# gruai/koifish

Measured on AMD Instinct MI355X. Metric: tokens/sec/GPU Qwen3 4-bit prefill+decode; achieved HBM GB/s vs peak, higher is better.
Workload: dtype u4 weights x bf16, fp32 accumulate; 1 GPU; Qwen3-0.6B 4-bit PackedQ greedy decode, 1xMI355X per replica, seq=2048: prompt 128, timed positions 1996..2047; order=canonical: bit-exact vs the CPU oracle, lm_head=bf16, replicas=1

## Files before the change

koifish_amd/csrc/kf_abi.hip:

```cpp
#include <stdarg.h>
#include <stdio.h>
#include <string.h>


#include <mutex>
#include <math.h>
#include <stdlib.h>

#include <vector>

#include "kf_a8.h"
#include "kf_attn_plan.h"
#include "kf_attn_docs_plan.h"
#include "kf_gemm_plan.h"
#include "kf_gemv_plan.h"
#include "kf_gemv_rows_plan.h"
#include "kf_score_plan.h"
#include "kf_gama_plan.h"
#include "kf_lora_plan.h"
#include "kf_gradnorm_plan.h"
#include "kf_rowq.h"
#include "kf_engine_host.h"

struct kf_ctx {
// ... 1727 lines not shown
}
size_t kf_engine_head_screen_bytes(int vocab, int dim) { return kf::head_screen_bytes(vocab, dim); }
int kf_engine_set_head_screen(kf_ctx* c, kf_engine* e, void* buf, size_t bytes) {
    ENG_ENTER(c, e && e->h, "engine");
    ENG_NOT_CAPTURING(c);
    return ok_or(kf::engine_set_head_screen(e->h, buf, bytes, c->stream),
                 "kf_engine_set_head_screen: needs a head set by kf_engine_set_head and a 256-byte aligned buffer of kf_engine_head_screen_bytes(vocab, dim) bytes");
}
int kf_engine_screen_stats(kf_ctx* c, kf_engine* e, kf_engine_screen_statistics* out) {
    ENG_ENTER(c, e && e->h && out, "argument");
    long long w[3];
    ENG_HIP(kf::engine_screen_stats(e->h, c->stream, w));
    out->screened_steps = w[0], out->rows_reranked = w[1], out->wg_fallbacks = w[2];
    return KF_OK;
}
int kf_engine_reset(kf_ctx* c, kf_engine* e) {
    ENG_ENTER(c, e && e->h, "engine");
    ENG_NOT_CAPTURING(c);
    ENG_HIP(kf::eng_then_sync(KF_OK, c->stream));
    ENG_HIP(kf::engine_reset(e->h, c->stream));
    return KF_OK;
}
int kf_engine_set_embedding(kf_ctx* c, kf_engine* e, const kf_weight* embed_or_null, const int32_t* d_forced) {
    ENG_ENTER(c, e && e->h, "engine");
    ENG_NOT_CAPTURING(c);
    return ok_or(kf::engine_set_embedding(e->h, embed_or_null, d_forced),
                 "kf_engine_set_embedding: the fused row read takes a bf16 table of the engine's width (other storages keep kf_embed_state)");
}
int kf_engine_served(kf_ctx* c, const kf_engine_desc* d, char* why, size_t why_bytes) {
    CHKCTX(c);
    const char* w = "";
    const int rc = kf::engine_build(d, nullptr, 0, c->stream, nullptr, &w, kf::ENG_DRY);
    return eng_served(rc, __func__, w, why, why_bytes);
}
int kf_engine_tune(kf_ctx* c, kf_engine* e, kf_bf16* x_out, const int32_t* d_state, int pos_bound, int passes, float* us_before, float* us_after) {
    ENG_ENTER(c, e && e->h, "engine");
    ENG_NOT_CAPTURING(c);
    kf::engine_set_canonical(e->h, c->canonical);
    const int rc = kf::engine_tune(e->h, c->stream, x_out, d_state, pos_bound, passes, us_before, us_after);
    return rc < 0 ? fail(rc, "kf_engine_tune failed with %d (no embedding table set, or a poll timed out)", rc) : rc;
}
int kf_engine_stats(kf_ctx* c, kf_engine* e, int pos_bound, kf_engine_statistics* out) {
    ENG_ENTER(c, e && e->h && out, "argument");
    int w[14];
    ENG_HIP(kf::engine_stats(e->h, c->stream, pos_bound, w));
    for (int i = 0; i < 6; i++) out->sweeps[i] = w[i], out->delay[i] = w[7 + i];
    out->polls = w[6], out->tuned = w[13];
    return KF_OK;
}
int kf_engine_check(kf_ctx* c, kf_engine* e) {
    ENG_ENTER(c, e && e->h, "engine");
    int err = 0;
    ENG_HIP(kf::engine_error_word(e->h, c->stream, &err));
    if (err) return fail(KF_INTERNAL_ERR, "kf_engine: a hand-off poll timed out (error word 0x%x): the launch was not fully resident", err);
    return KF_OK;
}
size_t kf_xengine_workspace_bytes(const kf_engine_desc* d) { return d ? kf::xengine_ws_bytes(d) : 0; }
int kf_xengine_create(kf_ctx* c, const kf_engine_desc* d, int n_seq, int64_t kv_seq_stride, void* ws, size_t ws_bytes, kf_xengine** out) {
    ENG_ENTER(c, d && ws && out, "argument");
    ENG_NOT_CAPTURING(c);
    if (n_seq < 1 || n_seq > KF_XENGINE_MAX_SEQ) return fail(KF_INVALID_ARGS, "kf_xengine_create: n_seq %d outside 1 .. %d (up to four sequences per XCD)", n_seq, KF_XENGINE_MAX_SEQ);
    kf::XEngineHost* h = nullptr;
    const char* why = "";
    const int rc = kf::xengine_build(d, n_seq, (long long)kv_seq_stride, ws, ws_bytes, c->stream, &h, &why);
    return ENG_WRAP(kf_xengine, rc, why, h, out);
}
size_t kf_xengine_workspace_bytes_tp(const kf_engine_desc* d) { return d ? kf::xengine_ws_bytes_tp(d) : 0; }
int kf_xengine_create_tp(kf_ctx* c, const kf_engine_desc* const* ds, int world, void* ws, size_t ws_bytes, kf_xengine** out) {
    ENG_ENTER(c, ds && ws && out, "argument");
    ENG_NOT_CAPTURING(c);
    kf::XEngineHost* h = nullptr;
    const char* why = "";
    const int rc = kf::xengine_build_tp(ds, world, ws, ws_bytes, c->stream, &h, &why);
    return ENG_WRAP(kf_xengine, rc, why, h, out);
}
int kf_xengine_set_head_tp(kf_ctx* c, kf_xengine* e, const kf_weight* const* shards, const int32_t* row0, const kf_bf16* final_norm_w, kf_bf16* logits, int32_t* d_tokens_out, int tokens_stride) {
    ENG_ENTER(c, e && e->h, "engine");
    return ok_or(kf::xengine_set_head_tp(e->h, shards, row0, final_norm_w, logits, d_tokens_out, tokens_stride),
                 "kf_xengine_set_head_tp: eight bf16 [rows, dim] vocabulary shards in rank order (row0 = the rows before), a norm weight and a logits buffer");
}
int kf_xengine_served(kf_ctx* c, const kf_engine_desc* d, char* why, size_t why_bytes) {
    CHKCTX(c);
    if (!d) return fail(KF_INVALID_ARGS, "kf_xengine_served: null descriptor");
    const char* w = "";
    const int rc = kf::xengine_build(d, 1, 0, nullptr, 0, c->stream, nullptr, &w, kf::ENG_DRY);
    return eng_served(rc, __func__, w, why, why_bytes);
}
int kf_xengine_set_embedding(kf_ctx* c, kf_xengine* e, const kf_weight* embed, const int32_t* d_forced, int forced_stride) {
    ENG_ENTER(c, e && e->h && embed, "argument");
    if (d_forced && forced_stride < 1) return fail(KF_INVALID_ARGS, "kf_xengine_set_embedding: forced_stride %d", forced_stride);
    return ok_or(kf::xengine_set_embedding(e->h, embed, d_forced, forced_stride), "kf_xengine_set_embedding: the row read inside the launch takes a bf16 table of the engine's width");
}
int kf_xengine_set_head(kf_ctx* c, kf_xengine* e, const kf_weight* head_or_null, const kf_bf16* final_norm_w, kf_bf16* logits, int32_t* d_tokens_out, int tokens_stride) {
    ENG_ENTER(c, e && e->h, "engine");
    return ok_or(kf::xengine_set_head(e->h, head_or_null, final_norm_w, logits, d_tokens_out, tokens_stride),
                 "kf_xengine_set_head: the in-launch head takes a bf16 [vocab, dim] matrix of the engine's width, a norm weight and a logits buffer");
}
int kf_xengine_steps(kf_ctx* c, kf_xengine* e, kf_bf16* x_out, int32_t* d_state, int n_steps, int pick) {
    ENG_ENTER(c, e && e->h, "engine");
    if (!c->canonical) return fail(KF_UNSUPPORTED_DATATYPE, "kf_xengine_steps: the XCD-confined engines run the canonical summation order only (kf_set_canonical(ctx, 1))");
    if (n_steps < 1 || (n_steps > 1 && !pick)) return fail(KF_INVALID_ARGS, "kf_xengine_steps: n_steps %d (several steps per launch need the pick inside)", n_steps);
    if (c->capturing) return fail(KF_INVALID_ARGS, "kf_xengine_steps: not while capturing (the launch's generation is a kernel argument the host counts: a replayed launch would repeat it)");
    const int rc = kf::xengine_steps(e->h, c->stream, d_state, x_out, pick ? 2 : 1, n_steps);
    if (rc == KF_UNSUPPORTED_DATATYPE) return fail(rc, "kf_xengine_steps: the form for this many sequences does not fit the LDS at this depth");
    return rc == KF_OK ? KF_OK : fail(rc, "kf_xengine_steps failed with %d (no embedding / head set?)", rc);
}
// ... 212 lines not shown
```

koifish_amd/csrc/kf_attn_common.h:

```cpp
#pragma once
#include "kf_kernels.h"

namespace kf {

__device__ __forceinline__ float group_sum16(float v, int lg) {
    if (lg >= 1) v += dpp_f<0xB1>(v);
    if (lg >= 2) v += dpp_f<0x4E>(v);
    if (lg >= 3) v += dpp_f<0x141>(v);
    if (lg >= 4) v += dpp_f<0x140>(v);
    return v;
}
struct HeadRaw {
    uint16_t x0, x1, w0, w1;
};
__device__ __forceinline__ HeadRaw load_head(const uint16_t* __restrict__ src, const uint16_t* __restrict__ wn, int hd) {
    const int half = hd >> 1;
    int j = threadIdx.x & 63;
    j = j < half ? j : half - 1;
    const uint16_t* w = wn ? wn : src;
    return HeadRaw{src[j], src[j + half], w[j], w[j + half]};
}
__device__ __forceinline__ void prep_head_cs(const HeadRaw r, bool norm, bool rope, float c, float sn, int hd, float eps, uint16_t* dst, float* rstd_out = nullptr, int lane_in = -1) {
    const int lane = lane_in >= 0 ? lane_in : (int)(threadIdx.x & 63), half = hd >> 1;
    const int j = lane;
    const bool act = j < half;
    float x0 = act ? bf2f(r.x0) : 0.f, x1 = act ? bf2f(r.x1) : 0.f;
    if (norm) {
        const float w0 = bf2f(r.w0), w1 = bf2f(r.w1);
        const double ss = wave_sum_f64_fast(fma((double)x0, (double)x0, (double)x1 * (double)x1));
        const float s0 = 1.0f / sqrtf((float)ss / (float)hd + eps);
        const float s = round_bf16(s0);
        if (rstd_out && lane == 0) *rstd_out = s0;
        x0 = round_bf16(x0 * s * w0);
        x1 = round_bf16(x1 * s * w1);
    }
    if (rope) {
        const float a = x0 * c, b = x1 * sn, cc = x0 * sn, d = x1 * c;
        x0 = round_bf16(a - b);
        x1 = round_bf16(cc + d);
    }
    if (act) dst[j] = f2bf(x0), dst[j + half] = f2bf(x1);
}
__device__ __forceinline__ void prep_head(const HeadRaw r, bool norm, const float* __restrict__ tab_pos, int hd, float eps, uint16_t* dst, float* rstd_out = nullptr) {
    const int j = threadIdx.x & 63;
    float c = 1.f, sn = 0.f;
    if (tab_pos && j < (hd >> 1)) c = tab_pos[2 * j], sn = tab_pos[2 * j + 1];
    prep_head_cs(r, norm, tab_pos != nullptr, c, sn, hd, eps, dst, rstd_out);
}

__device__ __forceinline__ float fast_exp(float x) { return __builtin_amdgcn_exp2f(x * 1.44269502162933349609375f); }

constexpr int ATTN_U = 4;

struct AttnAt { int pos, t1; bool empty; };
template <int GQ, int NW, int HD, int EL>
struct AttnSlice {
    static constexpr int hd_log2 = HD == 128 ? 7 : 6;
    static constexpr int LPK = HD / EL, KPW = 64 / LPK, lpk_log2 = hd_log2 - (EL == 16 ? 4 : 3), tstride = NW * KPW, NQ = (GQ + NW - 1) / NW;
    const int gq_split, split, kvh, gpart, chunk, t0;
    __device__ __forceinline__ AttnSlice(int gq_split_, int chunk_)
        : gq_split(gq_split_), split(blockIdx.x), kvh((int)blockIdx.y / gq_split), gpart((int)blockIdx.y - kvh * gq_split), chunk(chunk_), t0(split * chunk) {}
    __device__ __forceinline__ int h0() const { return (kvh * gq_split + gpart) * GQ; }
    __device__ __forceinline__ int tstart(int wave, int grp) const { return t0 + wave * KPW + grp; }
    __device__ __forceinline__ int end(int last) const {
        int t = t0 + chunk;
        if (t > last + 1) t = last + 1;
        return t;
    }
    __device__ __forceinline__ AttnAt at(const int* d_pos, int pos_bound) const {
        const int pos = d_pos ? *d_pos : pos_bound, len = pos + 1;
        return AttnAt{pos, end(pos), t0 >= len};
    }
    __device__ __forceinline__ bool holds(int pos, int t1) const { return (pos >= t0) && (pos < t1); }
};

constexpr float KF_LOG2E = 1.44269502162933349609375f;
__device__ __forceinline__ float canon_score(const float (&q)[8], u32x4 kw, int lpk_log2, float rden) {
    const uint32_t k4[4] = {kw.x, kw.y, kw.z, kw.w};
    float d = 0.f;
#pragma unroll
    for (int i = 0; i < 4; i++) {
        d = fmaf(q[2 * i], bf_lo(k4[i]), d);
        d = fmaf(q[2 * i + 1], bf_hi(k4[i]), d);
    }
    d = group_sum16(d, lpk_log2);
    return round_bf16(d * rden);
}
__device__ __forceinline__ int canon_shift(float d) { return (int)fmaxf(d, -1022.0f); }
__device__ __forceinline__ double ldexp_d(double v, int e) { return __builtin_ldexp(v, e); }
__device__ __forceinline__ double swap32_add_d(double a, double b) {
    const unsigned long long ua = __builtin_bit_cast(unsigned long long, a), ub = __builtin_bit_cast(unsigned long long, b);
    const auto lo = __builtin_amdgcn_permlane32_swap((unsigned)ua, (unsigned)ub, false, false);
    const auto hi = __builtin_amdgcn_permlane32_swap((unsigned)(ua >> 32), (unsigned)(ub >> 32), false, false);
    return __builtin_bit_cast(double, ((unsigned long long)hi[0] << 32) | lo[0]) + __builtin_bit_cast(double, ((unsigned long long)hi[1] << 32) | lo[1]);
}
__device__ __forceinline__ double swap16_add_d(double a, double b) {
    const unsigned long long ua = __builtin_bit_cast(unsigned long long, a), ub = __builtin_bit_cast(unsigned long long, b);
    const auto lo = __builtin_amdgcn_permlane16_swap((unsigned)ua, (unsigned)ub, false, false);
    const auto hi = __builtin_amdgcn_permlane16_swap((unsigned)(ua >> 32), (unsigned)(ub >> 32), false, false);
    return __builtin_bit_cast(double, ((unsigned long long)hi[0] << 32) | lo[0]) + __builtin_bit_cast(double, ((unsigned long long)hi[1] << 32) | lo[1]);
}
template <int GQ>
struct CanonAcc {
    double o[GQ][8], l[GQ];
    float m[GQ];
    __device__ __forceinline__ void init() {
#pragma unroll
        for (int hq = 0; hq < GQ; hq++) {
            m[hq] = -__builtin_inff(), l[hq] = 0.0;
#pragma unroll
            for (int i = 0; i < 8; i++) o[hq][i] = 0.0;
        }
    }
};
template <int K>
__device__ __forceinline__ uint32_t row_bcast_u(uint32_t v) {
    return (uint32_t)__builtin_amdgcn_update_dpp(0, (int)v, 0x150 + K, 0xF, 0xF, true);
}
template <int K>
__device__ __forceinline__ float row_bcast_f(float v) { return __uint_as_float(row_bcast_u<K>(__float_as_uint(v))); }
template <int K>
__device__ __forceinline__ double row_bcast_d(double v) {
    const unsigned long long u = __builtin_bit_cast(unsigned long long, v);
    return __builtin_bit_cast(double, ((unsigned long long)row_bcast_u<K>((uint32_t)(u >> 32)) << 32) | row_bcast_u<K>((uint32_t)u));
}
__device__ __forceinline__ float canon_dot(const float (&q)[8], u32x4 kw, int lpk_log2) {
    const uint32_t k4[4] = {kw.x, kw.y, kw.z, kw.w};
    float d = 0.f;
#pragma unroll
// ... 78 lines not shown
        const double p = vmine ? ldexp_d((double)f, canon_shift(n - m_mine)) : 0.0;
        double vd[U][8];
#pragma unroll
        for (int u = 0; u < U; u++) {
            const uint32_t vw[4] = {vv[u].x, vv[u].y, vv[u].z, vv[u].w};
#pragma unroll
            for (int i = 0; i < 4; i++) vd[u][2 * i] = (double)bf_lo(vw[i]), vd[u][2 * i + 1] = (double)bf_hi(vw[i]);
        }
        canon_apply_items<GQ, U>(A, p, vd);
        return;
    }
    float f[U][GQ], n[U][GQ], bn[GQ];
#pragma unroll
    for (int hq = 0; hq < GQ; hq++) bn[hq] = -__builtin_inff();
#pragma unroll
    for (int u = 0; u < U; u++) {
#pragma unroll
        for (int hq = 0; hq < GQ; hq++) {
            const float s = canon_score(qf[hq], kk[u], lpk_log2, rden);
            kf_exp2_parts(s * KF_LOG2E, f[u][hq], n[u][hq]);
            n[u][hq] = valid[u] ? n[u][hq] : -__builtin_inff();
            bn[hq] = fmaxf(bn[hq], n[u][hq]);
        }
    }
#pragma unroll
    for (int hq = 0; hq < GQ; hq++) {
        bn[hq] = xmax32(xmax16(bn[hq]));
        if (LPK < 16) bn[hq] = fmaxf(bn[hq], dpp_f<0x128>(bn[hq]));
        if (bn[hq] > A.m[hq]) {
            if (A.m[hq] > -__builtin_inff()) {
                const int e = canon_shift(A.m[hq] - bn[hq]);
                A.l[hq] = ldexp_d(A.l[hq], e);
#pragma unroll
                for (int i = 0; i < 8; i++) A.o[hq][i] = ldexp_d(A.o[hq][i], e);
            }
            A.m[hq] = bn[hq];
        }
    }
#pragma unroll
    for (int u = 0; u < U; u++) {
        const uint32_t vw[4] = {vv[u].x, vv[u].y, vv[u].z, vv[u].w};
        double vd[8];
#pragma unroll
        for (int i = 0; i < 4; i++) vd[2 * i] = (double)bf_lo(vw[i]), vd[2 * i + 1] = (double)bf_hi(vw[i]);
#pragma unroll
        for (int hq = 0; hq < GQ; hq++) {
            const double p = valid[u] ? ldexp_d((double)f[u][hq], canon_shift(n[u][hq] - A.m[hq])) : 0.0;
            A.l[hq] += p;
#pragma unroll
            for (int i = 0; i < 8; i++) A.o[hq][i] = fma(p, vd[i], A.o[hq][i]);
        }
    }
}
template <int GQ, int LPK>
__device__ __forceinline__ void canon_wave_to_lds(const CanonAcc<GQ>& A, double* comb_wave , int hd, int lane, int d0) {
    const int row = lane >> 4;
#pragma unroll
    for (int hq = 0; hq < GQ; hq++) {
        double s1[4], r2[2];
#pragma unroll
        for (int i = 0; i < 4; i++) s1[i] = swap32_add_d(A.o[hq][i], A.o[hq][i + 4]);
#pragma unroll
        for (int i = 0; i < 2; i++) {
            r2[i] = swap16_add_d(s1[i], s1[i + 2]);
            if (LPK < 16) r2[i] += dpp_d<0x128>(r2[i]);
        }
        double lt = xsum16_d(xsum32_d(A.l[hq]));
        if (LPK < 16) lt += dpp_d<0x128>(lt);
        double* c = comb_wave + (size_t)hq * (hd + 2);
        if (LPK == 16 || (lane & 8) == 0) c[d0 + 2 * row] = r2[0], c[d0 + 2 * row + 1] = r2[1];
        if (lane == 0) c[hd] = lt, c[hd + 1] = (double)A.m[hq];
    }
}

template <int GQ, int NW, int HD>
__device__ __forceinline__ void canon_slice_publish(const double* comb, double* part, uint16_t* odst, int h0, int nsp, int split) {
    constexpr int hd = HD, hd_log2 = HD == 128 ? 7 : 6, PS = hd + 2;
    for (int i = threadIdx.x; i < GQ * hd; i += blockDim.x) {
        const int hq = i >> hd_log2, d = i & (hd - 1);
        float ms = -__builtin_inff();
#pragma unroll
        for (int sl = 0; sl < NW; sl++) ms = fmaxf(ms, (float)comb[((size_t)sl * GQ + hq) * PS + hd + 1]);
        double o = 0.0, L = 0.0;
#pragma unroll
        for (int sl = 0; sl < NW; sl++) {
            const double* c = comb + ((size_t)sl * GQ + hq) * PS;
            const int e = canon_shift((float)c[hd + 1] - ms);
            o += ldexp_d(c[d], e);
            L += ldexp_d(c[hd], e);
        }
        if (nsp == 1) {
            odst[(size_t)(h0 + hq) * hd + d] = f2bf((float)(o / L));
        } else {
            double* dst = part + ((size_t)(h0 + hq) * nsp + split) * PS;
            __hip_atomic_store(dst + d, o, __ATOMIC_RELAXED, __HIP_MEMORY_SCOPE_AGENT);
            if (d == 0) __hip_atomic_store(dst + hd, L, __ATOMIC_RELAXED, __HIP_MEMORY_SCOPE_AGENT), __hip_atomic_store(dst + hd + 1, (double)ms, __ATOMIC_RELAXED, __HIP_MEMORY_SCOPE_AGENT);
        }
    }
}
template <int GQ, int HD>
__device__ __forceinline__ void canon_slice_publish_empty(double* part, int h0, int nsp, int split) {
    constexpr int hd = HD, hd_log2 = HD == 128 ? 7 : 6, PS = hd + 2;
    for (int i = threadIdx.x; i < GQ * hd; i += blockDim.x) {
        const int hq = i >> hd_log2, d = i & (hd - 1);
        double* dst = part + ((size_t)(h0 + hq) * nsp + split) * PS;
        __hip_atomic_store(dst + d, 0.0, __ATOMIC_RELAXED, __HIP_MEMORY_SCOPE_AGENT);
        if (d == 0) __hip_atomic_store(dst + hd, 0.0, __ATOMIC_RELAXED, __HIP_MEMORY_SCOPE_AGENT), __hip_atomic_store(dst + hd + 1, -(double)__builtin_inff(), __ATOMIC_RELAXED, __HIP_MEMORY_SCOPE_AGENT);
    }
}
template <int GQ, int NW, int HD>
__device__ __forceinline__ void canon_arrive_and_merge(const double* part, int* counter, int* flag, uint16_t* odst, int h0, int nsp) {
    constexpr int hd = HD, hd_log2 = HD == 128 ? 7 : 6, PS = hd + 2;
    const int tid = threadIdx.x, lane = tid & 63;
    asm volatile("s_waitcnt vmcnt(0)" ::: "memory");
    __syncthreads();
    if (tid == 0) {
        const int old = __hip_atomic_fetch_add(counter, 1, __ATOMIC_RELAXED, __HIP_MEMORY_SCOPE_AGENT);
        flag[0] = (old == nsp - 1);
    }
    __syncthreads();
    if (!flag[0]) return;
    constexpr int NT = NW * 64;
    constexpr int NV = (GQ * 128 + NT - 1) / NT;
#pragma unroll
// ... 134 lines not shown
```

koifish_amd/csrc/kf_engine.hip:

```cpp
#include <stdlib.h>
#include <string.h>

#include <vector>

#include <type_traits>

#include "kf_attn_plan.h"
#include "kf_engine_common.h"
#include "kf_engine_host.h"

namespace kf {


struct EngXOff {
    int xA, qkv, ao, xB, act, part, hbest, tokg, end;
};
constexpr EngXOff eng_xoff(int dim, int qd, int kvd, int ffn, int hd) {
    EngXOff o{};
    o.xA = 0, o.qkv = o.xA + eng_gran_dw(dim), o.ao = o.qkv + eng_gran_dw(qd + 2 * kvd), o.xB = o.ao + eng_gran_dw(qd), o.act = o.xB + eng_gran_dw(dim);
    o.part = o.act + eng_gran_dw(ffn);
    o.hbest = o.part + eng_gran_dw(2 * (qd / hd) * KF_ATTN_MAX_SPLITS * (2 * hd + 4));
    o.tokg = o.hbest + eng_gran_dw(2 * ENG_NWG);
    o.end = o.tokg + eng_gran_dw(2);
    return o;
// ... 337 lines not shown
        T.kk[u] = T.vv[u] = u32x4{0, 0, 0, 0};
        if (t < S.t1) {
            const size_t off = (size_t)t * a.kv_stride + (size_t)S.kvh * hd + d0;
            T.kk[u] = *reinterpret_cast<const u32x4 KF_GLOBAL*>(ly.kcache + off);
            T.vv[u] = *reinterpret_cast<const u32x4 KF_GLOBAL*>(ly.vcache + off);
        }
    }
}
template <class C>
__device__ __forceinline__ void eng_attn_phase(const EngArgs& a, const EngLds& L, const EngSlice& S, const EngLayer& ly, uint32_t gen, uint32_t tag, int wave, int lane,
                                               EngAttnState<C>& T, int l, int wg) {
    constexpr bool DBG = C::DBG;
    constexpr int GQ = C::GQ, hd = C::HD, hd_log2 = C::HD == 128 ? 7 : 6, LPK = hd >> 3, KPW = 64 / LPK, lpk_log2 = hd_log2 - 3, NWA = C::NWV, U = EngAttnState<C>::U;
    constexpr bool XMAP = C::XMAP;
    constexpr int NQ = (GQ + NWA - 1) / NWA;
    const int tid = (wave << 6) | lane, pos = S.pos, nsp = S.nsp, kvh = S.kvh, h0 = S.h0, t1 = S.t1;
    const int grp = lane >> lpk_log2, d0 = (lane & (LPK - 1)) * 8;
    const int tstride = NWA * KPW, tstart = S.t0 + wave * KPW + grp;
    const int nbatch = (S.t1 - S.t0 + U * tstride - 1) / (U * tstride);
    __syncthreads();
    if (wave == 0) ENG_STAMP(1, 2);
    if (!S.empty) {
        {
            const bool rope = a.rope_table != nullptr;
            const bool qnorm = ly.norm_q != nullptr;
            const int half = hd >> 1, j = lane < half ? lane : half - 1;
#pragma unroll
            for (int i = 0; i < NQ; i++) {
                const int hq = wave + i * NWA;
                if (hq < GQ) {
                    HeadRaw r;
                    r.x0 = L.qraw[hq * hd + j], r.x1 = L.qraw[hq * hd + j + half];
                    r.w0 = qnorm ? T.nw0 : r.x0, r.w1 = qnorm ? T.nw1 : r.x1;
                    prep_head_cs(r, qnorm, rope, T.rc, T.rs, hd, a.qk_eps, L.qb + hq * hd, nullptr, lane);
                }
            }
            if (S.own_new && wave == (GQ % NWA)) {
                HeadRaw r;
                r.x0 = L.kraw[j], r.x1 = L.kraw[j + half];
                r.w0 = ly.norm_k ? T.nw0 : r.x0, r.w1 = ly.norm_k ? T.nw1 : r.x1;
                prep_head_cs(r, ly.norm_k != nullptr, rope, T.rc, T.rs, hd, a.qk_eps, L.knew, nullptr, lane);
            }
        }
        __syncthreads();
        if (wave == 0) ENG_STAMP(1, 11);
        if (S.own_new) {
            g_u16w krow = ly.kcache + (size_t)pos * a.kv_stride + (size_t)kvh * hd;
            g_u16w vrow = ly.vcache + (size_t)pos * a.kv_stride + (size_t)kvh * hd;
            if (tid < hd / 8) {
                *reinterpret_cast<u32x4 KF_GLOBAL*>(const_cast<uint16_t KF_GLOBAL*>(krow) + 8 * tid) = *reinterpret_cast<const u32x4*>(L.knew + 8 * tid);
                *reinterpret_cast<u32x4 KF_GLOBAL*>(const_cast<uint16_t KF_GLOBAL*>(vrow) + 8 * tid) = *reinterpret_cast<const u32x4*>(L.vraw + 8 * tid);
            }
        }
        using Acc = std::conditional_t<C::CANON, CanonAcc<GQ>, FastAcc<GQ>>;
        using Sum = std::conditional_t<C::CANON, double, float>;
        Acc A;
        A.init();
        float qf[GQ][8];
        u32x4 qp[GQ];
#pragma unroll
        for (int hq = 0; hq < GQ; hq++) {
            const u32x4 qv = *reinterpret_cast<const u32x4*>(L.qb + hq * hd + d0);
            const uint32_t q4[4] = {qv.x, qv.y, qv.z, qv.w};
            qp[hq] = qv;
#pragma unroll
            for (int i = 0; i < 4; i++) qf[hq][2 * i] = bf_lo(q4[i]), qf[hq][2 * i + 1] = bf_hi(q4[i]);
        }
        const float rden = 1.0f / sqrtf((float)hd);
        for (int b = 0; b < nbatch; b++) {
            const int tb = tstart + b * U * tstride;
            u32x4 ck[U], cv[U];
            bool valid[U];
#pragma unroll
            for (int u = 0; u < U; u++) {
                const int t = tb + u * tstride;
                valid[u] = t < t1;
                ck[u] = T.kk[u], cv[u] = T.vv[u];
                if (valid[u] && t == pos) ck[u] = *reinterpret_cast<const u32x4*>(L.knew + d0), cv[u] = *reinterpret_cast<const u32x4*>(L.vraw + d0);
            }
            if (b + 1 < nbatch) eng_attn_issue<C>(a, ly, S, wave, lane, T, b + 1);
            if constexpr (C::CANON) canon_batch<GQ, LPK, U>(A, qf, ck, cv, valid, lpk_log2, rden);
            else fast_batch<GQ, LPK, U>(A, qp, ck, cv, valid, lpk_log2, rden);
        }
        if (wave == 0) ENG_STAMP(1, 12);
        Sum* const comb = reinterpret_cast<Sum*>(L.comb);
        if constexpr (C::CANON) canon_wave_to_lds<GQ, LPK>(A, comb + (size_t)wave * GQ * (hd + 2), hd, lane, d0);
        else fast_wave_to_lds<GQ, LPK>(A, comb + (size_t)wave * GQ * (hd + 2), hd, lane, d0);
        if (wave == 0) ENG_STAMP(1, 13);
        __syncthreads();
        if (wave == 0) ENG_STAMP(1, 14);
        constexpr int PSD = hd + 2;
        for (int i = tid; i < GQ * hd; i += NWA * 64) {
            const int hq = i >> hd_log2, d = i & (hd - 1);
            float ms = -__builtin_inff();
#pragma unroll
            for (int sl = 0; sl < NWA; sl++) ms = fmaxf(ms, (float)comb[((size_t)sl * GQ + hq) * PSD + hd + 1]);
            double o, Ls;
            if constexpr (C::CANON) {
                o = 0.0, Ls = 0.0;
#pragma unroll
                for (int sl = 0; sl < NWA; sl++) {
                    const double* c = L.comb + ((size_t)sl * GQ + hq) * PSD;
                    const int e = canon_shift((float)c[hd + 1] - ms);
                    o += ldexp_d(c[d], e);
                    Ls += ldexp_d(c[hd], e);
                }
            } else {
                float of = 0.f, lf = 0.f;
#pragma unroll
                for (int sl = 0; sl < NWA; sl++) {
                    const float* c = comb + ((size_t)sl * GQ + hq) * PSD;
                    const int e = fast_shift(c[hd + 1] - ms);
                    of += __builtin_ldexpf(c[d], e);
                    lf += __builtin_ldexpf(c[hd], e);
                }
                o = (double)of, Ls = (double)lf;
            }
            if (nsp == 1) {
                st_gran(a.xch + C::ao + (h0 + hq) * hd + d, tag, f2bf((float)(o / Ls)));
            } else {
                constexpr int ME = C::ME, MAXSP = KF_ATTN_MAX_SPLITS;
                const size_t oi = ((size_t)(d / ME) * (MAXSP * ME) + (size_t)S.split * ME + (d & (ME - 1))) * 2, mi = (size_t)hd * MAXSP * 2 + (size_t)S.split * 4;
                const unsigned long long ob = __builtin_bit_cast(unsigned long long, o), lb = __builtin_bit_cast(unsigned long long, Ls), gg = (unsigned long long)gen << 32;
                if (XMAP) {
                    unsigned long long* dst = eng_lpart<C>(a, S.xcc) + (size_t)hq * C::PSH;
                    *reinterpret_cast<ulonglong2*>(dst + oi) = ulonglong2{gg | (ob & 0xffffffffull), gg | (ob >> 32)};
                    if (d == 0) {
                        *reinterpret_cast<ulonglong2*>(dst + mi) = ulonglong2{gg | __float_as_uint(ms), gg | (lb & 0xffffffffull)};
                        dst[mi + 2] = gg | (lb >> 32);
                    }
                } else {
                    unsigned long long* dst = reinterpret_cast<unsigned long long*>(a.xch + C::part) + (size_t)(h0 + hq) * C::PSH;
                    st_gran64(dst + oi, gen, __uint_as_float((uint32_t)ob)), st_gran64(dst + oi + 1, gen, __uint_as_float((uint32_t)(ob >> 32)));
                    if (d == 0) st_gran64(dst + mi, gen, ms), st_gran64(dst + mi + 1, gen, __uint_as_float((uint32_t)lb)), st_gran64(dst + mi + 2, gen, __uint_as_float((uint32_t)(lb >> 32)));
                }
            }
        }
    } else if (nsp > 1) {
        for (int i = tid; i < GQ * hd; i += NWA * 64) {
            const int hq = i >> hd_log2, d = i & (hd - 1);
            constexpr int ME = C::ME, MAXSP = KF_ATTN_MAX_SPLITS;
            const size_t oi = ((size_t)(d / ME) * (MAXSP * ME) + (size_t)S.split * ME + (d & (ME - 1))) * 2, mi = (size_t)hd * MAXSP * 2 + (size_t)S.split * 4;
            const unsigned long long gg = (unsigned long long)gen << 32;
            if (XMAP) {
                unsigned long long* dst = eng_lpart<C>(a, S.xcc) + (size_t)hq * C::PSH;
                dst[oi] = gg, dst[oi + 1] = gg;
                if (d == 0) dst[mi] = gg | 0xff800000u, dst[mi + 1] = gg, dst[mi + 2] = gg;
            } else {
                unsigned long long* dst = reinterpret_cast<unsigned long long*>(a.xch + C::part) + (size_t)(h0 + hq) * C::PSH;
                st_gran64(dst + oi, gen, 0.f), st_gran64(dst + oi + 1, gen, 0.f);
                if (d == 0) st_gran64(dst + mi, gen, -__builtin_inff()), st_gran64(dst + mi + 1, gen, 0.f), st_gran64(dst + mi + 2, gen, 0.f);
            }
        }
    }
}

template <class C>
__device__ __forceinline__ void eng_poller_main(const EngArgs& a, const EngLds& L, const EngSlice& S, int epoch, int step, int wg, int lane) {
    using SH = typename C::SH;
    using P1 = typename SH::P1;
    using P4 = typename SH::P4;
    using P5 = typename SH::P5;
    using P6 = typename SH::P6;
    constexpr int FMT = C::FMT, GQ = C::GQ, HD = C::HD, NWV = C::NWV;
    constexpr bool XMAP = C::XMAP, DBG = C::DBG;
    constexpr int ND = C::DIM / 256, NQD = C::QD / 256, NF = C::FFN / 256;
    constexpr int XCH = C::XCH, hd = HD, hd_log2 = HD == 128 ? 7 : 6;
    bool dead = false;
    const bool has1 = XMAP ? true : wg * P1::spg < P1::total, has4 = wg * P4::spg < P4::total, has5 = wg * P5::spg < P5::total, has6 = wg * P6::spg < P6::total;
    constexpr int PW = eng_poller_role<NWV>();
    constexpr int NCW1 = ENG_P1_SHARE ? NWV : NWV - 1, S1 = c_maxs<P1, NCW1>(), NWP1 = P1::spg < NCW1 ? P1::spg : NCW1;
    constexpr bool P1_SHARE = ENG_P1_SHARE && P1::spg >= NWV;
    const float qb1 = S.j1 == 0 ? a.qbias[0] : (S.j1 == 1 ? a.qbias[1] : a.qbias[2]);
    const int row0_1 = S.s1 * P1::RPS;
    MvRegs<false, S1> r1;
    auto mat1 = [&](int l) {
        return L.lay[l].m[S.j1];
    };
    if (P1_SHARE) mv_prefetch<P1, NCW1, FMT, S1>(mat1(0), mat1(0), S.s1, PW, lane, S.M1, r1);
    EngAttnState<C> T;
#pragma unroll
    for (int u = 0; u < EngAttnState<C>::U; u++) T.kk[u] = T.vv[u] = u32x4{0, 0, 0, 0};
    eng_attn_rope<C>(a, S, lane, T);
    if (S.has_unit && !S.empty) eng_attn_issue<C>(a, L.lay[0], S, PW, lane, T, 0);
    int sw[4] = {0, 0, 0, 0};
    int swt[6] = {0, 0, 0, 0, 0, 0};
    for (int l = 0; l < a.n_layer; l++) {
        const EngLayer& ly = L.lay[l];
        const uint32_t gen = (uint32_t)epoch * (uint32_t)a.n_layer + (uint32_t)l, tag = gen & 0xffffu;
        if (S.has_unit && !S.empty) eng_attn_normw<C>(ly, PW, lane, T);
        MvPhase<C, P1, NCW1, S1> w1;
        if (P1_SHARE) w1.ahead(qb1, 0.f, PW, lane, r1, L.q1tab);
        ENG_STAMP(0, 0);
        ENG_PRIO_UP();
        if (has1 || has4) {
            if (l == 0) {
                const uint16_t* x0 = a.x_in;
                if (!x0) {
                    int tok = a.d_state[0];
                    if (step > 0) {
                        const __amdgpu_buffer_rsrc_t rt = eng_rsrc(a.xch + C::tokg, 8u);
                        for (int spins = 0;; spins++) {
                            const u32x2 g = __builtin_bit_cast(u32x2, __builtin_amdgcn_raw_buffer_load_b64(rt, 0, 0, 16 ));
                            if (g.y == (uint32_t)epoch) {
// ... 47 lines not shown
                for (int r = 0; r < NLQ; r++) g[r] = __builtin_bit_cast(u32x4, __builtin_amdgcn_raw_buffer_load_b128(rs, (q_src + 4 * (r * 64 + lane)) * 4, 0, 16));
                gk = __builtin_bit_cast(u32x4, __builtin_amdgcn_raw_buffer_load_b128(rs, (kv_in ? kv_src : 0) * 4, 0, 16));
#pragma unroll
                for (int r = 0; r < NLQ; r++) bad = (4 * (r * 64 + lane) < GQ * hd) ? tags_bad(g[r], tagw, bad) : bad;
                bad = kv_in ? tags_bad(gk, tagw, bad) : bad;
                if (all_good(bad)) {
                    swt[1] += spins + 1;
                    break;
                }
                if (dead || spins > ENG_SPIN_MAX) {
                    if (!dead && lane == 0) atomicOr(a.ws + 1, 2);
                    dead = true;
                    break;
                }
                __builtin_amdgcn_s_sleep(1);
            }
#pragma unroll
            for (int r = 0; r < NLQ; r++) {
                const int e0 = 4 * (r * 64 + lane);
                if (e0 < GQ * hd) *reinterpret_cast<u32x2*>(L.qraw + e0) = u32x2{(g[r].x & 0xffffu) | (g[r].y << 16), (g[r].z & 0xffffu) | (g[r].w << 16)};
            }
            if (kv_in) *reinterpret_cast<u32x2*>(L.kraw + e_kv) = u32x2{(gk.x & 0xffffu) | (gk.y << 16), (gk.z & 0xffffu) | (gk.w << 16)};
            ENG_STAMP(0, 2);
            if (P1_SHARE) {
                const int ln = l + 1 < a.n_layer ? l + 1 : l;
                mv_prefetch<P1, NCW1, FMT, S1>(mat1(ln), mat1(ln), S.s1, PW, lane, S.M1, r1);
            }
            eng_attn_phase<C>(a, L, S, ly, gen, tag, PW, lane, T, l, wg);
            if (!S.empty) eng_attn_issue<C>(a, L.lay[l + 1 < a.n_layer ? l + 1 : l], S, PW, lane, T, 0);
        } else if (P1_SHARE) {
            const int ln = l + 1 < a.n_layer ? l + 1 : l;
            mv_prefetch<P1, NCW1, FMT, S1>(mat1(ln), mat1(ln), S.s1, PW, lane, S.M1, r1);
        }
        ENG_STAMP(0, 3);
        if (S.has_merge) {
            constexpr int ME = C::ME, NLM = C::NLM, MAXSP = KF_ATTN_MAX_SPLITS;
            const int nsp = S.nsp, h = S.me0 >> hd_log2, dd = S.me0 & (hd - 1);
            const unsigned long long* hbase = XMAP ? eng_lpart<C>(a, S.xcc) + (size_t)h * C::PSH : reinterpret_cast<const unsigned long long*>(a.xch + C::part) + (size_t)h * C::PSH;
            const __amdgpu_buffer_rsrc_t rs_o = eng_rsrc(hbase + (size_t)(dd / ME) * (MAXSP * ME * 2), (uint32_t)(MAXSP * ME * 2) * 8u);
            const __amdgpu_buffer_rsrc_t rs_ml = eng_rsrc(hbase + (size_t)hd * MAXSP * 2, (uint32_t)MAXSP * 32u);
            const int cnt = nsp * ME;
            u32x4 go[NLM], gm0, gm1;
            const bool mine = lane < nsp;
            eng_wait_pub(nullptr, 0, a.delay[2], dead);
            ENG_STAMP(0, 9);
            ENG_PRIO_UP();
            int msw = 0;
            for (int spins = 0;; spins++) {
                uint32_t bad = 0;
                msw = spins + 1;
#pragma unroll
                for (int r = 0; r < NLM; r++) go[r] = __builtin_bit_cast(u32x4, __builtin_amdgcn_raw_buffer_load_b128(rs_o, (r * 64 + lane) * 16, 0, 16 ));
                gm0 = __builtin_bit_cast(u32x4, __builtin_amdgcn_raw_buffer_load_b128(rs_ml, (mine ? lane : 0) * 32, 0, 16));
                gm1 = __builtin_bit_cast(u32x4, __builtin_amdgcn_raw_buffer_load_b128(rs_ml, (mine ? lane : 0) * 32 + 16, 0, 16));
#pragma unroll
                for (int r = 0; r < NLM; r++) bad |= (r * 64 + lane) < cnt ? ((go[r].y ^ gen) | (go[r].w ^ gen)) : 0u;
                bad |= mine ? ((gm0.y ^ gen) | (gm0.w ^ gen) | (gm1.y ^ gen)) : 0u;
                if (all_good(bad)) break;
                if (dead || spins > ENG_SPIN_MAX) {
                    if (!dead && lane == 0) atomicOr(a.ws + 1, 4);
                    dead = true;
                    break;
                }
                __builtin_amdgcn_s_sleep(1);
            }
            ENG_STAMP(0, 11);
            swt[2] += msw;
            if (DBG && wg == a.dbg_wg && lane == 0) a.dbg[((size_t)l * 2) * 16 + 10] = (unsigned long long)msw;
#pragma unroll
            for (int r = 0; r < NLM; r++) {
                const int vi = r * 64 + lane;
                if (vi < MAXSP * ME) {
                    const int sp = vi / ME, e = vi - sp * ME;
                    L.msc[e * MAXSP + sp] = vi < cnt ? __builtin_bit_cast(double, ((unsigned long long)go[r].z << 32) | go[r].x) : 0.0;
                }
            }
            const float ms = mine ? __uint_as_float(gm0.x) : -__builtin_inff();
            const double ls = mine ? __builtin_bit_cast(double, ((unsigned long long)gm1.x << 32) | gm0.z) : 0.0;
            const float Mx = wave_max(ms);
            const int sh = canon_shift(ms - Mx);
            const double Lt = wave_sum_f64_fast(ldexp_d(ls, sh));
            int* shl = reinterpret_cast<int*>(L.msc + ME * MAXSP + 32);
            if (lane < MAXSP) shl[lane] = sh;
            double o = 0.0;
            {
                constexpr int QS = MAXSP / 4;
                const int e = (4 * ME <= 64) ? (lane >> 2) : lane, qq = (4 * ME <= 64) ? (lane & 3) : 0;
                const bool on = e < ME;
                const double* mv = L.msc + (on ? e : 0) * MAXSP + qq * QS;
                const int* sv = shl + qq * QS;
                if (4 * ME <= 64) {
#pragma unroll
                    for (int k = 0; k < QS; k++) o += ldexp_d(mv[k], sv[k]);
                    o += dpp_d<0xB1>(o);
                    o += dpp_d<0x4E>(o);
                } else {
#pragma unroll
                    for (int k = 0; k < MAXSP; k++) o += ldexp_d(mv[k], shl[k]);
                }
            }
            const uint32_t gr = (tag << 16) | (uint32_t)f2bf((float)(o / Lt));
            const bool holder = (4 * ME <= 64) ? ((lane & 3) == 0 && (lane >> 2) < ME) : (lane < ME);
            const int he = (4 * ME <= 64) ? (lane >> 2) : lane;
            uint32_t* const ao_dst = a.xch + C::ao + (XMAP ? S.h0 * hd : 0) + S.me0;
            if (ME >= 4) {
                uint32_t* mo = reinterpret_cast<uint32_t*>(L.msc + ME * MAXSP);
                if (holder) mo[he] = gr;
                if (4 * lane < ME) __builtin_amdgcn_raw_buffer_store_b128(*reinterpret_cast<const u32x4*>(mo + 4 * lane), eng_rsrc(ao_dst, (uint32_t)ME * 4u), lane * 16, 0, 16 );
            } else if (holder) {
                __hip_atomic_store(ao_dst + he, gr, __ATOMIC_RELAXED, __HIP_MEMORY_SCOPE_AGENT);
            }
            ENG_PRIO_DOWN();
        }
        ENG_STAMP(0, 4);
        if (ENG_COOP) {
            if (has4) eng_wait_pub(nullptr, 0, a.delay[3], dead);
            __syncthreads();
            if (has4) eng_poll_stage_part<XCH, NQD, P4::nBlk, NWV, C::F32X>(a.xch + C::ao, tag, L.xs[1], PW, lane, a.ws, dead, &sw[1]);
        } else if (has4) {
            eng_poll_stage<XCH, NQD, P4::nBlk, false, false, C::F32X>(a.xch + C::ao, nullptr, tag, nullptr, 0.f, L.xs[1], nullptr, lane, a.ws, dead, &sw[1], nullptr, 0, a.delay[3]);
        }
        ENG_STAMP(0, 5);
        __syncthreads();
        ENG_PRIO_UP();
        if (has5 || has6)
            eng_poll_stage<XCH, ND, P5::nBlk, true, false, C::F32X>(a.xch + C::xB, nullptr, tag, ly.norm_post, a.eps, L.xs[0], L.xrawB, lane, a.ws, dead, &sw[2], has4 ? L.pub + 1 : nullptr, l + 1,
                                                           a.delay[4]);
        ENG_PRIO_DOWN();
        ENG_STAMP(0, 6);
        __syncthreads();
        if (ENG_COOP) {
            if (has6) eng_wait_pub(has5 ? L.pub + 2 : nullptr, l + 1, a.delay[5], dead);
            __syncthreads();
            if (has6) eng_poll_stage_part<XCH, NF, P6::nBlk, NWV, C::F32X>(a.xch + C::act, tag, L.xs[1], PW, lane, a.ws, dead, &sw[3]);
        } else if (has6) {
            eng_poll_stage<XCH, NF, P6::nBlk, false, false, C::F32X>(a.xch + C::act, nullptr, tag, nullptr, 0.f, L.xs[1], nullptr, lane, a.ws, dead, &sw[3], has5 ? L.pub + 2 : nullptr, l + 1, a.delay[5]);
        }
        ENG_STAMP(0, 7);
        swt[0] += sw[0], swt[3] += sw[1], swt[4] += sw[2], swt[5] += sw[3];
        if (DBG && wg == a.dbg_wg && lane == 0)
            a.dbg[((size_t)l * 2) * 16 + 8] = (unsigned long long)sw[0] | ((unsigned long long)sw[1] << 16) | ((unsigned long long)sw[2] << 32) | ((unsigned long long)sw[3] << 48);
        __syncthreads();
    }
    if (wg == 0 && lane == 0) {
#pragma unroll
        for (int i = 0; i < 6; i++) atomicAdd(a.ws + 8 + i, swt[i]);
        atomicAdd(a.ws + 14, a.n_layer);
    }
}

template <class C>
// ... 906 lines not shown
```

Measured before the change: 2418 tokens/s.

## Use fixed-exponent canonical attention accumulation, dropping running-max rescaling

Canonical (bit-exact) attention in the persistent engine now accumulates exp terms scaled by their own absolute exponent in double precision, with no running max. This removes the max exchange, the per-split shift computation and the ldexp rescaling in both the intra-block and cross-split combines, and shrinks the published partial metadata by one word. Scores whose exponent exceeds a fixed limit set an error bit, and the host reports that the per-layer path must be used instead. The risk is exactness: it relies on double-precision sums of absolutely scaled terms matching the oracle within that range.

```diff
diff --git a/koifish_amd/csrc/kf_abi.hip b/koifish_amd/csrc/kf_abi.hip
--- a/koifish_amd/csrc/kf_abi.hip
+++ b/koifish_amd/csrc/kf_abi.hip
@@ -1803,6 +1803,8 @@
     ENG_ENTER(c, e && e->h, "engine");
     int err = 0;
     ENG_HIP(kf::engine_error_word(e->h, c->stream, &err));
+    if (err & 128)
+        return fail(KF_INTERNAL_ERR, "kf_engine: attention scores outside the engine's fixed-exponent range (error word 0x%x): the per-layer launches serve such a model (set_engine(False))", err);
     if (err) return fail(KF_INTERNAL_ERR, "kf_engine: a hand-off poll timed out (error word 0x%x): the launch was not fully resident", err);
     return KF_OK;
 }
diff --git a/koifish_amd/csrc/kf_attn_common.h b/koifish_amd/csrc/kf_attn_common.h
--- a/koifish_amd/csrc/kf_attn_common.h
+++ b/koifish_amd/csrc/kf_attn_common.h
@@ -1,4 +1,6 @@
 #pragma once
+#include <type_traits>
+
 #include "kf_kernels.h"
 
 namespace kf {
@@ -75,6 +77,7 @@
 };
 
 constexpr float KF_LOG2E = 1.44269502162933349609375f;
+constexpr float KF_CANON_FIX_LIM = 448.0f;
 __device__ __forceinline__ float canon_score(const float (&q)[8], u32x4 kw, int lpk_log2, float rden) {
     const uint32_t k4[4] = {kw.x, kw.y, kw.z, kw.w};
     float d = 0.f;
@@ -259,8 +262,49 @@
         }
     }
 }
-template <int GQ, int LPK>
-__device__ __forceinline__ void canon_wave_to_lds(const CanonAcc<GQ>& A, double* comb_wave , int hd, int lane, int d0) {
+template <int GQ>
+struct CanonAccFixed {
+    double o[GQ][8], l[GQ];
+    bool oob;
+    __device__ __forceinline__ void init() {
+        oob = false;
+#pragma unroll
+        for (int hq = 0; hq < GQ; hq++) {
+            l[hq] = 0.0;
+#pragma unroll
+            for (int i = 0; i < 8; i++) o[hq][i] = 0.0;
+        }
+    }
+};
+template <int GQ, int LPK, int U = ATTN_U>
+__device__ __forceinline__ void canon_batch_fixed(CanonAccFixed<GQ>& A, const float (&qf)[GQ][8], const u32x4 (&kk)[U], const u32x4 (&vv)[U], const bool (&valid)[U], int lpk_log2, float rden) {
+    float f[U][GQ], n[U][GQ];
+#pragma unroll
+    for (int u = 0; u < U; u++) {
+#pragma unroll
+        for (int hq = 0; hq < GQ; hq++) {
+            const float s = canon_score(qf[hq], kk[u], lpk_log2, rden);
+            kf_exp2_parts(s * KF_LOG2E, f[u][hq], n[u][hq]);
+            A.oob |= valid[u] && !(fabsf(n[u][hq]) <= KF_CANON_FIX_LIM);
+        }
+    }
+#pragma unroll
+    for (int u = 0; u < U; u++) {
+        const uint32_t vw[4] = {vv[u].x, vv[u].y, vv[u].z, vv[u].w};
+        double vd[8];
+#pragma unroll
+        for (int i = 0; i < 4; i++) vd[2 * i] = (double)bf_lo(vw[i]), vd[2 * i + 1] = (double)bf_hi(vw[i]);
+#pragma unroll
+        for (int hq = 0; hq < GQ; hq++) {
+            const double p = valid[u] ? ldexp_d((double)f[u][hq], (int)n[u][hq]) : 0.0;
+            A.l[hq] += p;
+#pragma unroll
+            for (int i = 0; i < 8; i++) A.o[hq][i] = fma(p, vd[i], A.o[hq][i]);
+        }
+    }
+}
+template <int GQ, int LPK, class Acc>
+__device__ __forceinline__ void canon_wave_to_lds(const Acc& A, double* comb_wave , int hd, int lane, int d0) {
     const int row = lane >> 4;
 #pragma unroll
     for (int hq = 0; hq < GQ; hq++) {
@@ -276,7 +320,11 @@
         if (LPK < 16) lt += dpp_d<0x128>(lt);
         double* c = comb_wave + (size_t)hq * (hd + 2);
         if (LPK == 16 || (lane & 8) == 0) c[d0 + 2 * row] = r2[0], c[d0 + 2 * row + 1] = r2[1];
-        if (lane == 0) c[hd] = lt, c[hd + 1] = (double)A.m[hq];
+        if constexpr (std::is_same_v<Acc, CanonAccFixed<GQ>>) {
+            if (lane == 0) c[hd] = lt;
+        } else {
+            if (lane == 0) c[hd] = lt, c[hd + 1] = (double)A.m[hq];
+        }
     }
 }
 
diff --git a/koifish_amd/csrc/kf_engine.hip b/koifish_amd/csrc/kf_engine.hip
--- a/koifish_amd/csrc/kf_engine.hip
+++ b/koifish_amd/csrc/kf_engine.hip
@@ -413,7 +413,7 @@
                 *reinterpret_cast<u32x4 KF_GLOBAL*>(const_cast<uint16_t KF_GLOBAL*>(vrow) + 8 * tid) = *reinterpret_cast<const u32x4*>(L.vraw + 8 * tid);
             }
         }
-        using Acc = std::conditional_t<C::CANON, CanonAcc<GQ>, FastAcc<GQ>>;
+        using Acc = std::conditional_t<C::CANON, CanonAccFixed<GQ>, FastAcc<GQ>>;
         using Sum = std::conditional_t<C::CANON, double, float>;
         Acc A;
         A.init();
@@ -440,8 +440,11 @@
                 if (valid[u] && t == pos) ck[u] = *reinterpret_cast<const u32x4*>(L.knew + d0), cv[u] = *reinterpret_cast<const u32x4*>(L.vraw + d0);
             }
             if (b + 1 < nbatch) eng_attn_issue<C>(a, ly, S, wave, lane, T, b + 1);
-            if constexpr (C::CANON) canon_batch<GQ, LPK, U>(A, qf, ck, cv, valid, lpk_log2, rden);
+            if constexpr (C::CANON) canon_batch_fixed<GQ, LPK, U>(A, qf, ck, cv, valid, lpk_log2, rden);
             else fast_batch<GQ, LPK, U>(A, qp, ck, cv, valid, lpk_log2, rden);
+        }
+        if constexpr (C::CANON) {
+            if (__builtin_amdgcn_ballot_w64(A.oob) != 0 && lane == 0) atomicOr(a.ws + 1, 128);
         }
         if (wave == 0) ENG_STAMP(1, 12);
         Sum* const comb = reinterpret_cast<Sum*>(L.comb);
@@ -454,19 +457,18 @@
         for (int i = tid; i < GQ * hd; i += NWA * 64) {
             const int hq = i >> hd_log2, d = i & (hd - 1);
             float ms = -__builtin_inff();
-#pragma unroll
-            for (int sl = 0; sl < NWA; sl++) ms = fmaxf(ms, (float)comb[((size_t)sl * GQ + hq) * PSD + hd + 1]);
             double o, Ls;
             if constexpr (C::CANON) {
                 o = 0.0, Ls = 0.0;
 #pragma unroll
-                for (int sl = 0; sl < NWA; sl++) {
-                    const double* c = L.comb + ((size_t)sl * GQ + hq) * PSD;
-                    const int e = canon_shift((float)c[hd + 1] - ms);
-                    o += ldexp_d(c[d], e);
-                    Ls += ldexp_d(c[hd], e);
+                for (int sl = 0; sl < NWA; sl++) o += L.comb[((size_t)sl * GQ + hq) * PSD + d];
+                if (nsp == 1 || d == 0) {
+#pragma unroll
+                    for (int sl = 0; sl < NWA; sl++) Ls += L.comb[((size_t)sl * GQ + hq) * PSD + hd];
                 }
             } else {
+#pragma unroll
+                for (int sl = 0; sl < NWA; sl++) ms = fmaxf(ms, (float)comb[((size_t)sl * GQ + hq) * PSD + hd + 1]);
                 float of = 0.f, lf = 0.f;
 #pragma unroll
                 for (int sl = 0; sl < NWA; sl++) {
@@ -486,14 +488,20 @@
                 if (XMAP) {
                     unsigned long long* dst = eng_lpart<C>(a, S.xcc) + (size_t)hq * C::PSH;
                     *reinterpret_cast<ulonglong2*>(dst + oi) = ulonglong2{gg | (ob & 0xffffffffull), gg | (ob >> 32)};
-                    if (d == 0) {
+                    if constexpr (C::CANON) {
+                        if (d == 0) *reinterpret_cast<ulonglong2*>(dst + mi) = ulonglong2{gg | (lb & 0xffffffffull), gg | (lb >> 32)};
+                    } else if (d == 0) {
                         *reinterpret_cast<ulonglong2*>(dst + mi) = ulonglong2{gg | __float_as_uint(ms), gg | (lb & 0xffffffffull)};
                         dst[mi + 2] = gg | (lb >> 32);
                     }
                 } else {
                     unsigned long long* dst = reinterpret_cast<unsigned long long*>(a.xch + C::part) + (size_t)(h0 + hq) * C::PSH;
                     st_gran64(dst + oi, gen, __uint_as_float((uint32_t)ob)), st_gran64(dst + oi + 1, gen, __uint_as_float((uint32_t)(ob >> 32)));
-                    if (d == 0) st_gran64(dst + mi, gen, ms), st_gran64(dst + mi + 1, gen, __uint_as_float((uint32_t)lb)), st_gran64(dst + mi + 2, gen, __uint_as_float((uint32_t)(lb >> 32)));
+                    if constexpr (C::CANON) {
+                        if (d == 0) st_gran64(dst + mi, gen, __uint_as_float((uint32_t)lb)), st_gran64(dst + mi + 1, gen, __uint_as_float((uint32_t)(lb >> 32)));
+                    } else if (d == 0) {
+                        st_gran64(dst + mi, gen, ms), st_gran64(dst + mi + 1, gen, __uint_as_float((uint32_t)lb)), st_gran64(dst + mi + 2, gen, __uint_as_float((uint32_t)(lb >> 32)));
+                    }
                 }
             }
         }
@@ -506,11 +514,19 @@
             if (XMAP) {
                 unsigned long long* dst = eng_lpart<C>(a, S.xcc) + (size_t)hq * C::PSH;
                 dst[oi] = gg, dst[oi + 1] = gg;
-                if (d == 0) dst[mi] = gg | 0xff800000u, dst[mi + 1] = gg, dst[mi + 2] = gg;
+                if constexpr (C::CANON) {
+                    if (d == 0) dst[mi] = gg, dst[mi + 1] = gg;
+                } else if (d == 0) {
+                    dst[mi] = gg | 0xff800000u, dst[mi + 1] = gg, dst[mi + 2] = gg;
+                }
             } else {
                 unsigned long long* dst = reinterpret_cast<unsigned long long*>(a.xch + C::part) + (size_t)(h0 + hq) * C::PSH;
                 st_gran64(dst + oi, gen, 0.f), st_gran64(dst + oi + 1, gen, 0.f);
-                if (d == 0) st_gran64(dst + mi, gen, -__builtin_inff()), st_gran64(dst + mi + 1, gen, 0.f), st_gran64(dst + mi + 2, gen, 0.f);
+                if constexpr (C::CANON) {
+                    if (d == 0) st_gran64(dst + mi, gen, 0.f), st_gran64(dst + mi + 1, gen, 0.f);
+                } else if (d == 0) {
+                    st_gran64(dst + mi, gen, -__builtin_inff()), st_gran64(dst + mi + 1, gen, 0.f), st_gran64(dst + mi + 2, gen, 0.f);
+                }
             }
         }
     }
@@ -664,10 +680,11 @@
 #pragma unroll
                 for (int r = 0; r < NLM; r++) go[r] = __builtin_bit_cast(u32x4, __builtin_amdgcn_raw_buffer_load_b128(rs_o, (r * 64 + lane) * 16, 0, 16 ));
                 gm0 = __builtin_bit_cast(u32x4, __builtin_amdgcn_raw_buffer_load_b128(rs_ml, (mine ? lane : 0) * 32, 0, 16));
-                gm1 = __builtin_bit_cast(u32x4, __builtin_amdgcn_raw_buffer_load_b128(rs_ml, (mine ? lane : 0) * 32 + 16, 0, 16));
+                if constexpr (!C::CANON) gm1 = __builtin_bit_cast(u32x4, __builtin_amdgcn_raw_buffer_load_b128(rs_ml, (mine ? lane : 0) * 32 + 16, 0, 16));
 #pragma unroll
                 for (int r = 0; r < NLM; r++) bad |= (r * 64 + lane) < cnt ? ((go[r].y ^ gen) | (go[r].w ^ gen)) : 0u;
-                bad |= mine ? ((gm0.y ^ gen) | (gm0.w ^ gen) | (gm1.y ^ gen)) : 0u;
+                if constexpr (C::CANON) bad |= mine ? ((gm0.y ^ gen) | (gm0.w ^ gen)) : 0u;
+                else bad |= mine ? ((gm0.y ^ gen) | (gm0.w ^ gen) | (gm1.y ^ gen)) : 0u;
                 if (all_good(bad)) break;
                 if (dead || spins > ENG_SPIN_MAX) {
                     if (!dead && lane == 0) atomicOr(a.ws + 1, 4);
@@ -687,28 +704,48 @@
                     L.msc[e * MAXSP + sp] = vi < cnt ? __builtin_bit_cast(double, ((unsigned long long)go[r].z << 32) | go[r].x) : 0.0;
                 }
             }
-            const float ms = mine ? __uint_as_float(gm0.x) : -__builtin_inff();
-            const double ls = mine ? __builtin_bit_cast(double, ((unsigned long long)gm1.x << 32) | gm0.z) : 0.0;
-            const float Mx = wave_max(ms);
-            const int sh = canon_shift(ms - Mx);
-            const double Lt = wave_sum_f64_fast(ldexp_d(ls, sh));
-            int* shl = reinterpret_cast<int*>(L.msc + ME * MAXSP + 32);
-            if (lane < MAXSP) shl[lane] = sh;
-            double o = 0.0;
-            {
+            double o, Lt;
+            if constexpr (C::CANON) {
+                const double ls = mine ? __builtin_bit_cast(double, ((unsigned long long)gm0.z << 32) | gm0.x) : 0.0;
+                Lt = wave_sum_f64_fast(ls);
+                o = 0.0;
                 constexpr int QS = MAXSP / 4;
                 const int e = (4 * ME <= 64) ? (lane >> 2) : lane, qq = (4 * ME <= 64) ? (lane & 3) : 0;
                 const bool on = e < ME;
                 const double* mv = L.msc + (on ? e : 0) * MAXSP + qq * QS;
-                const int* sv = shl + qq * QS;
                 if (4 * ME <= 64) {
 #pragma unroll
-                    for (int k = 0; k < QS; k++) o += ldexp_d(mv[k], sv[k]);
+                    for (int k = 0; k < QS; k++) o += mv[k];
                     o += dpp_d<0xB1>(o);
                     o += dpp_d<0x4E>(o);
                 } else {
 #pragma unroll
-                    for (int k = 0; k < MAXSP; k++) o += ldexp_d(mv[k], shl[k]);
+                    for (int k = 0; k < MAXSP; k++) o += mv[k];
+                }
+            } else {
+                const float ms = mine ? __uint_as_float(gm0.x) : -__builtin_inff();
+                const double ls = mine ? __builtin_bit_cast(double, ((unsigned long long)gm1.x << 32) | gm0.z) : 0.0;
+                const float Mx = wave_max(ms);
+                const int sh = canon_shift(ms - Mx);
+                Lt = wave_sum_f64_fast(ldexp_d(ls, sh));
+                int* shl = reinterpret_cast<int*>(L.msc + ME * MAXSP + 32);
+                if (lane < MAXSP) shl[lane] = sh;
+                o = 0.0;
+                {
+                    constexpr int QS = MAXSP / 4;
+                    const int e = (4 * ME <= 64) ? (lane >> 2) : lane, qq = (4 * ME <= 64) ? (lane & 3) : 0;
+                    const bool on = e < ME;
+                    const double* mv = L.msc + (on ? e : 0) * MAXSP + qq * QS;
+                    const int* sv = shl + qq * QS;
+                    if (4 * ME <= 64) {
+#pragma unroll
+                        for (int k = 0; k < QS; k++) o += ldexp_d(mv[k], sv[k]);
+                        o += dpp_d<0xB1>(o);
+                        o += dpp_d<0x4E>(o);
+                    } else {
+#pragma unroll
+                        for (int k = 0; k < MAXSP; k++) o += ldexp_d(mv[k], shl[k]);
+                    }
                 }
             }
             const uint32_t gr = (tag << 16) | (uint32_t)f2bf((float)(o / Lt));
```

Result: faster. 2484 tokens/s (median of 6 runs) (+2.7%).
